# Acly/dlimgedit

Measured on AMD Instinct MI355X. Metric: images/sec encode+mask @1024x1024, higher is better.
Workload: dtype f16; 1 GPU; SAM vit_b encoder + 1 point prompt, 1 image(s)/GPU/step, 1024x1024 RGBA, inputs and masks resident in HBM; timed through the extension entry point dlimg_amd_encode_and_mask (device pointers in and out) -- the drop-in table itself, host buffers in and out, is `abi_path`; weights=seeded synthetic, lanes_per_gpu=4, lanes_fed_by_the_step_queue=3, requests_coalesced_per_pass=4, passes_queued_per_lane=2

## Files before the change

### dlimgedit_amd/csrc/kernels/attention_window.hip

```cpp
#include "device_common.hpp"
#include "kernels.hpp"

#include <algorithm>
#include <cstdio>
#include <cstdlib>
#include <mutex>
#include <string>
#include <vector>

namespace dlimg {
namespace {

constexpr int WS = 14;
constexpr int SLOTS = 224;
constexpr int NW = 5;
constexpr int GRID = 64;
constexpr int V_STRIDE = 96;
constexpr int G_STRIDE = 33;
typedef short short4_t __attribute__((ext_vector_type(4)));
typedef __attribute__((address_space(3))) short4_t lds_short4_t;

struct WinSlot { int token; bool dummy; bool pad; };

DLIMG_DEVICE WinSlot win_slot(int slot, int wy, int wx) {
    int ty = slot >> 4, tx = slot & 15;
    int gy = wy * WS + ty, gx = wx * WS + tx;
    WinSlot s;
    s.dummy = tx >= WS;
    s.pad = !s.dummy && (gy >= GRID || gx >= GRID);
    s.token = gy * GRID + gx;
    return s;
}

DLIMG_DEVICE int k_row(int slot) { const int tx = slot & 15; return (slot >> 4) * WS + (tx < WS ? tx : WS - 1); }

template <int HD>
__global__ __launch_bounds__(448, 4) void attention_window_kernel(const half_t* __restrict__ qkv,
                                                               const half_t* __restrict__ qkv_pad,
                                                               const half_t* __restrict__ rel_h,
                                                               const half_t* __restrict__ rel_w,
                                                               half_t* __restrict__ out, int heads,
                                                               unsigned long long* stamps_arg) {
#ifdef DLIMG_TUNING
    unsigned long long* const stamps = stamps_arg;
#else
    unsigned long long* const stamps = nullptr;
#endif
    unsigned long long tstamp[8] = {0, 0, 0, 0, 0, 0, 0, 0};
    auto stamp = [&](int i) { if (stamps) tstamp[i] = __builtin_amdgcn_s_memtime(); };
    stamp(0);
    constexpr int KS = HD / 16;
    constexpr int DT = (HD + 31) / 32;
    constexpr int K_STRIDE = HD + 8;
    constexpr int CHUNKS = HD / 8;
    static_assert(DT * 32 <= V_STRIDE, "head dimension tiles must fit the padded V row");

    extern __shared__ __attribute__((aligned(16))) char smem[];
    half_t* lds_k = reinterpret_cast<half_t*>(smem);
    half_t* lds_v = lds_k + WS * WS * K_STRIDE;
    float* lds_g = reinterpret_cast<float*>(smem);

    const int D = heads * HD;
    const int ld = 3 * D;
    const int head = blockIdx.x % heads;
    const int win = (blockIdx.x / heads) % (NW * NW);
    const int img = blockIdx.x / (heads * NW * NW);
    const int wy = win / NW, wx = win % NW;
    const half_t* base = qkv + (size_t)img * 4096 * ld;
    const int tid = threadIdx.x;
    const int lane = lane_id();
    const int wave = wave_id();
    const int hi = lane >> 5, l31 = lane & 31;

    const int token0 = wy * WS * GRID + wx * WS;
    const int qslot = wave * 32 + l31;
    const WinSlot qs = win_slot(qslot, wy, wx);
    const bool q_real = !qs.dummy && !qs.pad;
    half8_t qf[KS];
    {
        const half_t* qrow = base + (size_t)(q_real ? qs.token : token0) * ld + head * HD + hi * 8;
#pragma unroll
        for (int ks = 0; ks < KS; ++ks) qf[ks] = *reinterpret_cast<const half8_t*>(qrow + ks * 16);
    }
    half8_t rfh[KS], rfw[KS];
    {
        const int rrow = l31 < 2 * WS - 1 ? l31 : 2 * WS - 2;
#pragma unroll
        for (int ks = 0; ks < KS; ++ks) {
            rfh[ks] = *reinterpret_cast<const half8_t*>(rel_h + rrow * HD + ks * 16 + hi * 8);
            rfw[ks] = *reinterpret_cast<const half8_t*>(rel_w + rrow * HD + ks * 16 + hi * 8);
        }
    }
    static_assert((SLOTS * CHUNKS) % 448 == 0, "K/V chunks split evenly over the workgroup");
    constexpr int KV_IT = SLOTS * CHUNKS / 448;
#if defined(DLIMG_TUNING) && defined(DLIMG_WINDOW_KV_EARLY)
    constexpr int KV_EARLY = HD == 64 ? KV_IT : DLIMG_WINDOW_KV_EARLY;
#else
    constexpr int KV_EARLY = HD == 64 ? KV_IT : 3;
#endif
    half8_t kreg[KV_IT], vreg[KV_IT];
    auto request_kv = [&](int it) {
        const int idx = tid + it * 448;
        const WinSlot ws = win_slot(idx / CHUNKS, wy, wx);
        const half_t* row = (ws.pad ? qkv_pad : base + (size_t)(ws.dummy ? token0 : ws.token) * ld) + head * HD + (idx % CHUNKS) * 8;
        kreg[it] = *reinterpret_cast<const half8_t*>(row + D);
        vreg[it] = *reinterpret_cast<const half8_t*>(row + 2 * D);
    };
#pragma unroll
    for (int it = 0; it < KV_EARLY; ++it) request_kv(it);
    __builtin_amdgcn_sched_barrier(0);
    stamp(1);
#pragma unroll
    for (int ks = 0; ks < KS; ++ks) {
        if (!q_real) qf[ks] = zero_h8();
        if (l31 >= 2 * WS - 1) { rfh[ks] = zero_h8(); rfw[ks] = zero_h8(); }
    }

    float* g = lds_g + wave * 32 * G_STRIDE;
    const int ty_q = qslot >> 4, tx_q = qslot & 15;
    float bh[WS];
    float bw[8];
    {
        float16_t acc = zero16();
#pragma unroll
        for (int ks = 0; ks < KS; ++ks) acc = mfma32(rfh[ks], qf[ks], acc);
#pragma unroll
        for (int r = 0; r < 16; ++r) g[l31 * G_STRIDE + acc_row(r, hi)] = acc[r];
        __builtin_amdgcn_sched_barrier(0);
        float16_t acc_w = zero16();
#pragma unroll
        for (int ks = 0; ks < KS; ++ks) acc_w = mfma32(rfw[ks], qf[ks], acc_w);
        if (KV_EARLY < KV_IT) {
            __builtin_amdgcn_sched_barrier(0);
#pragma unroll
            for (int it = KV_EARLY; it < KV_IT; ++it) request_kv(it);
            __builtin_amdgcn_sched_barrier(0);
        }
        __builtin_amdgcn_fence(__ATOMIC_RELEASE, "wavefront");
        __builtin_amdgcn_wave_barrier();
#pragma unroll
        for (int ky = 0; ky < WS; ++ky) bh[ky] = g[l31 * G_STRIDE + ty_q + (WS - 1) - ky] * sqrtf((float)HD);
        __builtin_amdgcn_fence(__ATOMIC_RELEASE, "wavefront");
        __builtin_amdgcn_wave_barrier();
#pragma unroll
        for (int r = 0; r < 16; ++r) g[l31 * G_STRIDE + acc_row(r, hi)] = acc_w[r];
        __builtin_amdgcn_fence(__ATOMIC_RELEASE, "wavefront");
        __builtin_amdgcn_wave_barrier();
#pragma unroll
        for (int e = 0; e < 8; ++e) {
            const int tx = (e & 3) + 8 * (e >> 2) + 4 * hi;
            bw[e] = tx < WS ? g[l31 * G_STRIDE + tx_q + (WS - 1) - tx] * sqrtf((float)HD) : -INFINITY;
        }
        __syncthreads();
    }
    stamp(2);

#pragma unroll
    for (int it = 0; it < KV_IT; ++it) {
        const int idx = tid + it * 448;
        const int slot = idx / CHUNKS, ch = idx % CHUNKS;
        const bool dummy = (slot & 15) >= WS;
        if (!dummy) *reinterpret_cast<half8_t*>(lds_k + k_row(slot) * K_STRIDE + ch * 8) = kreg[it];
        *reinterpret_cast<half8_t*>(lds_v + slot * V_STRIDE + ch * 8) = dummy ? zero_h8() : vreg[it];
    }
    if (DT * 32 > HD) {
        constexpr int PADC = (DT * 32 - HD) / 8;
        for (int idx = tid; idx < SLOTS * PADC; idx += 448)
            *reinterpret_cast<half8_t*>(lds_v + (idx / PADC) * V_STRIDE + HD + (idx % PADC) * 8) = zero_h8();
    }
    __syncthreads();
    stamp(3);

    const float scale = rsqrtf((float)HD);

    const half_t* kb = lds_k + k_row(l31) * K_STRIDE + hi * 8;
    auto score_tile = [&](int jt) {
        float16_t t;
#pragma unroll
        for (int r = 0; r < 16; ++r) {
            const int ty = jt * 2 + (r >> 3);
            const int e = (r & 3) + 4 * ((r >> 2) & 1);
            t[r] = bh[ty] + bw[e];
        }
#pragma unroll
        for (int ks = 0; ks < KS; ++ks) {
            half8_t kf = *reinterpret_cast<const half8_t*>(kb + (jt * 2 * WS) * K_STRIDE + ks * 16);
            t = mfma32(kf, qf[ks], t);
        }
        return t;
    };
#if defined(DLIMG_TUNING) && defined(DLIMG_WINDOW_TWO_PASS)
    constexpr bool ONLINE = false;
#else
    constexpr bool ONLINE = true;
#endif
    constexpr bool TWO_PASS = HD == 64 && !ONLINE;
    float16_t kept[(TWO_PASS || ONLINE) ? 1 : 7];
    float m = -INFINITY;
    const float c = scale * 1.44269504088896341f;
    if (!ONLINE) {
#pragma unroll
        for (int jt = 0; jt < 7; ++jt) {
            const float16_t t = score_tile(jt);
            if (!TWO_PASS) kept[jt] = t;
#pragma unroll
            for (int r = 0; r < 16; ++r) m = fmaxf(m, t[r]);
            __builtin_amdgcn_sched_barrier(0);
        }
        m = fmaxf(m, swap_halves(m));
    }
    stamp(4);
    float mc = -m * c;
    if (TWO_PASS) {
#pragma unroll
        for (int i = 0; i < WS; ++i) asm volatile("" : "+v"(bh[i]));
#pragma unroll
        for (int i = 0; i < 8; ++i) asm volatile("" : "+v"(bw[i]));
    }

    const half_t* vb = lds_v + ((hi * 4 + ((lane & 15) >> 2)) * V_STRIDE) + 16 * ((lane >> 4) & 1) + 4 * (lane & 3);
    float16_t o[DT];
#pragma unroll
    for (int dt = 0; dt < DT; ++dt) o[dt] = zero16();
    float l = 0.f;
#pragma unroll
    for (int jt = 0; jt < 7; ++jt) {
        float16_t t = (TWO_PASS || ONLINE) ? score_tile(jt) : kept[(TWO_PASS || ONLINE) ? 0 : jt];
        if (ONLINE) {
            float tm = fmaxf(fmaxf(t[0], t[1]), t[2]);
#pragma unroll
            for (int r = 3; r < 15; r += 2) tm = fmaxf(fmaxf(tm, t[r]), t[r + 1]);
            tm = fmaxf(tm, t[15]);
            tm = fmaxf(tm, swap_halves(tm));
            if (jt == 0) {
                m = tm;
                mc = -m * c;
            } else if (__any(__builtin_fmaf(tm, c, mc) > 8.0f)) {
                const float m_new = fmaxf(m, tm);
                const float alpha = __builtin_amdgcn_exp2f((m - m_new) * c);
#pragma unroll
                for (int dt = 0; dt < DT; ++dt)
#pragma unroll
                    for (int r = 0; r < 16; ++r) o[dt][r] *= alpha;
                l *= alpha;
                m = m_new;
                mc = -m * c;
            }
        }
#pragma unroll
        for (int r = 0; r < 16; ++r) {
            const float pv = __builtin_amdgcn_exp2f(__builtin_fmaf(t[r], c, mc));
            t[r] = pv;
            l += pv;
        }
#pragma unroll
        for (int st = 0; st < 2; ++st) {
            half8_t pf;
#pragma unroll
            for (int e = 0; e < 8; ++e) pf[e] = (half_t)t[st * 8 + e];
            const int key0 = jt * 32 + st * 16;
#pragma unroll
            for (int dt = 0; dt < DT; ++dt) {
                const half_t* vp = vb + key0 * V_STRIDE + dt * 32;
                const short4_t v0 = __builtin_amdgcn_ds_read_tr16_b64_v4i16((lds_short4_t*)vp);
                const short4_t v1 = __builtin_amdgcn_ds_read_tr16_b64_v4i16((lds_short4_t*)(vp + 8 * V_STRIDE));
                const half4_t h0 = __builtin_bit_cast(half4_t, v0), h1 = __builtin_bit_cast(half4_t, v1);
                half8_t vf = {h0[0], h0[1], h0[2], h0[3], h1[0], h1[1], h1[2], h1[3]};
                o[dt] = mfma32(vf, pf, o[dt]);
            }
        }
        __builtin_amdgcn_sched_barrier(0);
    }
    l += swap_halves(l);
    const float inv_l = 1.0f / l;
    stamp(5);

    __syncthreads();
    stamp(6);
    constexpr int ROWB = HD * 2 + 16;
    static_assert(7 * 32 * ROWB <= WS * WS * K_STRIDE * 2 + SLOTS * V_STRIDE * 2, "output slabs must fit in the K / V images");
    char* slab = smem + wave * 32 * ROWB;
#pragma unroll
    for (int dt = 0; dt < DT; ++dt)
#pragma unroll
        for (int g4 = 0; g4 < 4; ++g4) {
            const int d0 = dt * 32 + 8 * g4;
            if (d0 < HD) {
                const half4_t v = {(half_t)(o[dt][g4 * 4 + 0] * inv_l), (half_t)(o[dt][g4 * 4 + 1] * inv_l),
                                   (half_t)(o[dt][g4 * 4 + 2] * inv_l), (half_t)(o[dt][g4 * 4 + 3] * inv_l)};
                *reinterpret_cast<half4_t*>(slab + l31 * ROWB + hi * 8 + d0 * 2) = v;
            }
        }
    asm volatile("s_waitcnt lgkmcnt(0)" ::: "memory");
    constexpr int NIT = (32 * CHUNKS + 63) / 64;
#pragma unroll
    for (int it = 0; it < NIT; ++it) {
        const int idx = it * 64 + lane;
        const int row = idx / CHUNKS, ch = idx % CHUNKS;
        if (row < 32) {
            const WinSlot os = win_slot(wave * 32 + row, wy, wx);
            if (!os.dummy && !os.pad) {
                const float4_t v = *reinterpret_cast<const float4_t*>(slab + row * ROWB + ch * 16);
                store16_result(out + ((size_t)img * 4096 + os.token) * D + head * HD + ch * 8, v);
            }
        }
    }
    if (stamps && tid == 0) {
        asm volatile("s_waitcnt vmcnt(0)" ::: "memory");
        tstamp[7] = __builtin_amdgcn_s_memtime();
#pragma unroll
        for (int i = 0; i < 8; ++i) stamps[(size_t)blockIdx.x * 8 + i] = tstamp[i];
    }
}

template <int HD>
void launch_window(const half_t* qkv, const half_t* bias, const half_t* rel_h, const half_t* rel_w, half_t* out, int B,
                   int heads, hipStream_t s) {
    const size_t images = (size_t)WS * WS * (HD + 8) * 2 + (size_t)SLOTS * V_STRIDE * 2;
    const size_t scratch = 7 * 32 * G_STRIDE * 4;
    const size_t lds = images > scratch ? images : scratch;
    static k::LdsOptIn opt_in;
    opt_in.ensure((const void*)attention_window_kernel<HD>, lds, "attention_window: the device refuses the kernel's LDS size");
    unsigned long long* stamps = nullptr;
#ifdef DLIMG_TUNING
    static const bool want = std::getenv("DLIMGEDIT_WINDOW_STAMPS") != nullptr;
    static unsigned long long* buf = nullptr;
    const int wgs = B * NW * NW * heads;
    if (want) {
        if (!buf) (void)hipMalloc(&buf, (size_t)64 * NW * NW * 64 * 8 * sizeof(unsigned long long));
        if (wgs <= 64 * NW * NW * 64) stamps = buf;
    }
#endif
    hipLaunchKernelGGL(attention_window_kernel<HD>, dim3(B * NW * NW * heads), dim3(448), lds, s, qkv, bias, rel_h,
                       rel_w, out, heads, stamps);
#ifdef DLIMG_TUNING
    if (stamps) {
        static int launches = 0;
        if (++launches % 50 == 0) {
            (void)hipStreamSynchronize(s);
            std::vector<unsigned long long> h((size_t)wgs * 8);
            (void)hipMemcpy(h.data(), stamps, h.size() * sizeof(unsigned long long), hipMemcpyDeviceToHost);
            static const char* names[7] = {"requests", "rel-pos", "K/V->LDS", "pass 1", "pass 2", "barrier", "store"};
            std::string line = "[window stamps] " + std::to_string(wgs) + " workgroups, median cycles:";
            for (int p = 0; p < 7; ++p) {
                std::vector<unsigned long long> d(wgs);
                for (int w = 0; w < wgs; ++w) d[w] = h[(size_t)w * 8 + p + 1] - h[(size_t)w * 8 + p];
                std::nth_element(d.begin(), d.begin() + wgs / 2, d.end());
                line += std::string(" ") + names[p] + " " + std::to_string(d[wgs / 2]);
            }
            std::vector<unsigned long long> d(wgs);
            unsigned long long t0 = ~0ull, t1 = 0;
            for (int w = 0; w < wgs; ++w) { d[w] = h[(size_t)w * 8 + 7] - h[(size_t)w * 8]; t0 = std::min(t0, h[(size_t)w * 8]); t1 = std::max(t1, h[(size_t)w * 8 + 7]); }
            std::nth_element(d.begin(), d.begin() + wgs / 2, d.end());
            line += " | whole " + std::to_string(d[wgs / 2]) + " | first start to last end " + std::to_string(t1 - t0);
            fprintf(stderr, "%s\n", line.c_str());
        }
    }
#endif
}

}

namespace k {

void attention_window(const half_t* qkv, const half_t* qkv_pad, const half_t* rel_h, const half_t* rel_w, half_t* out,
                      int B, int heads, int hd, hipStream_t s) {
    if (B <= 0 || heads <= 0) throw_error("attention_window: empty problem");
    if (((uintptr_t)qkv | (uintptr_t)out | (uintptr_t)qkv_pad | (uintptr_t)rel_h | (uintptr_t)rel_w) & 15)
        throw_error("attention_window: buffers must be 16-byte aligned");
    switch (hd) {
    case 64: return launch_window<64>(qkv, qkv_pad, rel_h, rel_w, out, B, heads, s);
    case 80: return launch_window<80>(qkv, qkv_pad, rel_h, rel_w, out, B, heads, s);
    default: throw_error("attention_window: head dimension must be 64 or 80");
    }
}

}
}
```

Baseline: 878.5 images/s.

## Pack edge-window queries and skip idle waves in windowed attention

Query rows are remapped per window: in the last window column, where only 8 of 14 columns are real, each wave packs four 8-wide rows instead of two 16-wide rows. Waves that hold no real queries (from packing or from the short bottom window row) skip the bias, softmax and PV work and only help load K/V. The online-softmax rescale now decides per 16-lane group in packed windows, because each half-wave may serve a different query row. This cuts wasted MFMA work on padded edge windows, at the cost of extra branching and load imbalance across waves within a workgroup.

Result: no change. 880.6 images/s (median of 6 runs) (+0.2%).

```diff
diff --git a/dlimgedit_amd/csrc/kernels/attention_window.hip b/dlimgedit_amd/csrc/kernels/attention_window.hip
--- a/dlimgedit_amd/csrc/kernels/attention_window.hip
+++ b/dlimgedit_amd/csrc/kernels/attention_window.hip
@@ -30,6 +30,24 @@
     s.pad = !s.dummy && (gy >= GRID || gx >= GRID);
     s.token = gy * GRID + gx;
     return s;
+}
+
+struct WinQuery { int ty, tx, token; bool real; };
+
+DLIMG_DEVICE WinQuery win_query(int wave, int l, int wy, int wx) {
+    const bool packed = wx == NW - 1;
+    WinQuery q;
+    q.ty = packed ? wave * 4 + (l >> 3) : wave * 2 + (l >> 4);
+    q.tx = packed ? l & 7 : l & 15;
+    const int gy = wy * WS + q.ty, gx = wx * WS + q.tx;
+    q.real = q.ty < WS && q.tx < WS && gy < GRID && gx < GRID;
+    q.token = gy * GRID + gx;
+    return q;
+}
+
+DLIMG_DEVICE int win_active_waves(int wy, int wx) {
+    const int rows = wy == NW - 1 ? GRID - (NW - 1) * WS : WS;
+    return wx == NW - 1 ? (rows + 3) / 4 : (rows + 1) / 2;
 }
 
 DLIMG_DEVICE int k_row(int slot) { const int tx = slot & 15; return (slot >> 4) * WS + (tx < WS ? tx : WS - 1); }
@@ -71,11 +89,12 @@
     const int lane = lane_id();
     const int wave = wave_id();
     const int hi = lane >> 5, l31 = lane & 31;
+    const bool packed = wx == NW - 1;
+    const bool active = wave < win_active_waves(wy, wx);
 
     const int token0 = wy * WS * GRID + wx * WS;
-    const int qslot = wave * 32 + l31;
-    const WinSlot qs = win_slot(qslot, wy, wx);
-    const bool q_real = !qs.dummy && !qs.pad;
+    const WinQuery qs = win_query(wave, l31, wy, wx);
+    const bool q_real = qs.real;
     half8_t qf[KS];
     {
         const half_t* qrow = base + (size_t)(q_real ? qs.token : token0) * ld + head * HD + hi * 8;
@@ -110,32 +129,34 @@
     for (int it = 0; it < KV_EARLY; ++it) request_kv(it);
     __builtin_amdgcn_sched_barrier(0);
     stamp(1);
-#pragma unroll
-    for (int ks = 0; ks < KS; ++ks) {
-        if (!q_real) qf[ks] = zero_h8();
-        if (l31 >= 2 * WS - 1) { rfh[ks] = zero_h8(); rfw[ks] = zero_h8(); }
-    }
 
     float* g = lds_g + wave * 32 * G_STRIDE;
-    const int ty_q = qslot >> 4, tx_q = qslot & 15;
+    const int ty_q = qs.ty, tx_q = qs.tx;
     float bh[WS];
     float bw[8];
-    {
+    float16_t acc_w = zero16();
+    if (active) {
+#pragma unroll
+        for (int ks = 0; ks < KS; ++ks) {
+            if (!q_real) qf[ks] = zero_h8();
+            if (l31 >= 2 * WS - 1) { rfh[ks] = zero_h8(); rfw[ks] = zero_h8(); }
+        }
         float16_t acc = zero16();
 #pragma unroll
         for (int ks = 0; ks < KS; ++ks) acc = mfma32(rfh[ks], qf[ks], acc);
 #pragma unroll
         for (int r = 0; r < 16; ++r) g[l31 * G_STRIDE + acc_row(r, hi)] = acc[r];
         __builtin_amdgcn_sched_barrier(0);
-        float16_t acc_w = zero16();
 #pragma unroll
         for (int ks = 0; ks < KS; ++ks) acc_w = mfma32(rfw[ks], qf[ks], acc_w);
-        if (KV_EARLY < KV_IT) {
-            __builtin_amdgcn_sched_barrier(0);
-#pragma unroll
-            for (int it = KV_EARLY; it < KV_IT; ++it) request_kv(it);
-            __builtin_amdgcn_sched_barrier(0);
-        }
+    }
+    if (KV_EARLY < KV_IT) {
+        __builtin_amdgcn_sched_barrier(0);
+#pragma unroll
+        for (int it = KV_EARLY; it < KV_IT; ++it) request_kv(it);
+        __builtin_amdgcn_sched_barrier(0);
+    }
+    if (active) {
         __builtin_amdgcn_fence(__ATOMIC_RELEASE, "wavefront");
         __builtin_amdgcn_wave_barrier();
 #pragma unroll
@@ -151,8 +172,8 @@
             const int tx = (e & 3) + 8 * (e >> 2) + 4 * hi;
             bw[e] = tx < WS ? g[l31 * G_STRIDE + tx_q + (WS - 1) - tx] * sqrtf((float)HD) : -INFINITY;
         }
-        __syncthreads();
-    }
+    }
+    __syncthreads();
     stamp(2);
 
 #pragma unroll
@@ -195,6 +216,9 @@
     constexpr bool ONLINE = true;
 #endif
     constexpr bool TWO_PASS = HD == 64 && !ONLINE;
+    float16_t o[DT];
+    float inv_l = 0.f;
+    if (active) {
     float16_t kept[(TWO_PASS || ONLINE) ? 1 : 7];
     float m = -INFINITY;
     const float c = scale * 1.44269504088896341f;
@@ -219,7 +243,6 @@
     }
 
     const half_t* vb = lds_v + ((hi * 4 + ((lane & 15) >> 2)) * V_STRIDE) + 16 * ((lane >> 4) & 1) + 4 * (lane & 3);
-    float16_t o[DT];
 #pragma unroll
     for (int dt = 0; dt < DT; ++dt) o[dt] = zero16();
     float l = 0.f;
@@ -235,8 +258,10 @@
             if (jt == 0) {
                 m = tm;
                 mc = -m * c;
-            } else if (__any(__builtin_fmaf(tm, c, mc) > 8.0f)) {
-                const float m_new = fmaxf(m, tm);
+            } else if (const unsigned long long over = __ballot(__builtin_fmaf(tm, c, mc) > 8.0f)) {
+                const unsigned long long group = (lane & 16) ? 0xffff0000ffff0000ull : 0x0000ffff0000ffffull;
+                const bool raise = !packed || (over & group) != 0;
+                const float m_new = raise ? fmaxf(m, tm) : m;
                 const float alpha = __builtin_amdgcn_exp2f((m - m_new) * c);
 #pragma unroll
                 for (int dt = 0; dt < DT; ++dt)
@@ -272,11 +297,13 @@
         __builtin_amdgcn_sched_barrier(0);
     }
     l += swap_halves(l);
-    const float inv_l = 1.0f / l;
+    inv_l = 1.0f / l;
     stamp(5);
+    }
 
     __syncthreads();
     stamp(6);
+    if (active) {
     constexpr int ROWB = HD * 2 + 16;
     static_assert(7 * 32 * ROWB <= WS * WS * K_STRIDE * 2 + SLOTS * V_STRIDE * 2, "output slabs must fit in the K / V images");
     char* slab = smem + wave * 32 * ROWB;
@@ -298,12 +325,13 @@
         const int idx = it * 64 + lane;
         const int row = idx / CHUNKS, ch = idx % CHUNKS;
         if (row < 32) {
-            const WinSlot os = win_slot(wave * 32 + row, wy, wx);
-            if (!os.dummy && !os.pad) {
+            const WinQuery os = win_query(wave, row, wy, wx);
+            if (os.real) {
                 const float4_t v = *reinterpret_cast<const float4_t*>(slab + row * ROWB + ch * 16);
                 store16_result(out + ((size_t)img * 4096 + os.token) * D + head * HD + ch * 8, v);
             }
         }
+    }
     }
     if (stamps && tid == 0) {
         asm volatile("s_waitcnt vmcnt(0)" ::: "memory");
```
